# DecaYale/SYN3R

Measured on AMD Instinct MI355X. Metric: llff_3view_train_loop_iters_per_sec, higher is better.
Workload: dtype f32 raster / f16 UNet (f32 accumulate); 1 GPU; LLFF fern-like 3-view block: 50 raster fwd+bwd iters (l1 loss) (200000 Gaussians, 1920x1080, SH3) + 1 SVD (step,pass): CFG UNet fwd [2,14,8,72,128] f16 + fused Euler step; frames=14, parallelism=scene-parallel x1

## Files before the change

### syn3r_amd/csrc/raster_bin.hip

```cpp
#include "common.h"
#include "raster_common.h"

using namespace syn3r;

namespace syn3r {

size_t binning_bytes(long long P) {
    size_t n = (size_t)(P > 0 ? P : 1);
    return 2 * align256(n * 8) + 2 * align256(n * 4) + sort_scratch_bytes(n) + 256;
}

BinningState carve_binning(void* buf, long long P) {
    size_t n = (size_t)(P > 0 ? P : 1);
    char* p = (char*)buf;
    BinningState b;
    b.keys_a = (unsigned long long*)p; p += align256(n * 8);
    b.keys_b = (unsigned long long*)p; p += align256(n * 8);
    b.vals_a = (unsigned*)p; p += align256(n * 4);
    b.vals_b = (unsigned*)p; p += align256(n * 4);
    b.sort_scratch = p;
    return b;
}

}

namespace {

__global__ void __launch_bounds__(256) k_dup_tiles(int N, const unsigned* __restrict__ order,
                                                   const float* __restrict__ means2D, const int* __restrict__ radii,
                                                   const unsigned* __restrict__ offsets, int gx, int gy,
                                                   unsigned* __restrict__ keys, unsigned* __restrict__ vals,
                                                   unsigned cap, unsigned* __restrict__ header,
                                                   uint2* __restrict__ ranges, int tiles) {
    const int i = blockIdx.x * 256 + threadIdx.x;
    for (int t = i; t < tiles; t += gridDim.x * 256) ranges[t] = make_uint2(0u, 0u);
    const int lane = threadIdx.x & 63;
    const bool valid = i < N;
    unsigned id = valid ? order[i] : 0u;
    int r = valid ? radii[id] : 0;
    int x0 = 0, y0 = 0, x1 = 0, y1 = 0;
    if (r > 0) tile_rect(means2D[2 * (size_t)id], means2D[2 * (size_t)id + 1], r, gx, gy, x0, y0, x1, y1);
    const int w = x1 - x0;
    const unsigned cnt = (unsigned)(w * (y1 - y0));
    const unsigned incl = wave_scan_incl(cnt);
    const unsigned local = incl - cnt;
    const unsigned total = __shfl(incl, 63, 64);
    const int first = blockIdx.x * 256 + (threadIdx.x & ~63);
    const unsigned base = first < N ? offsets[first] : 0u;
    const float inv_w = w > 0 ? 1.0f / (float)w : 0.0f;
    for (unsigned t = 0; t < total; t += 64) {
        const unsigned p = t + lane;
        int j = 0;
#pragma unroll
        for (int step = 32; step > 0; step >>= 1) {
            unsigned lc = __shfl(local, j + step, 64);
            if (lc <= p) j += step;
        }
        const unsigned k = p - __shfl(local, j, 64);
        const int xj = __shfl(x0, j, 64), yj = __shfl(y0, j, 64), wj = __shfl(w, j, 64);
        const float iwj = __shfl(inv_w, j, 64);
        const unsigned idj = __shfl(id, j, 64);
        if (p < total) {
            const int ty = (int)(((float)k + 0.5f) * iwj);
            int tyc = ty;
            if ((unsigned)(tyc * wj) > k) --tyc;
            else if ((unsigned)((tyc + 1) * wj) <= k) ++tyc;
            const int tx = (int)k - tyc * wj;
            const unsigned o = base + p;
            if (o < cap) {
                keys[o] = (unsigned)((yj + tyc) * gx + xj + tx);
                vals[o] = idj;
            } else {
                header[1] = 1u;
// ... 491 lines not shown
```

### syn3r_amd/csrc/raster_bwd.hip

```cpp
#include "common.h"
#include "raster_common.h"

using namespace syn3r;

namespace {

constexpr int kGradSlots = 16;
enum { G_R = 0, G_G, G_B, G_DEPTH, G_MX, G_MY, G_CXX, G_CXY, G_CYY, G_OP, G_USED = 10 };

template <int NV>
__device__ __forceinline__ float reduce_lanes(float (&v)[10]) {
    static_assert(NV == 9 || NV == 10, "value 9 is the only optional one");
    float a[5];
#pragma unroll
    for (int k = 0; k < NV - 5; ++k) {
        auto r = __builtin_amdgcn_permlane32_swap(__float_as_int(v[k]), __float_as_int(v[k + 5]), false, false);
        a[k] = __int_as_float(r[0]) + __int_as_float(r[1]);
    }
    if (NV == 9) a[4] = v[4];
    float b[3];
#pragma unroll
    for (int k = 0; k < 2; ++k) {
        auto r = __builtin_amdgcn_permlane16_swap(__float_as_int(a[k]), __float_as_int(a[k + 3]), false, false);
        b[k] = __int_as_float(r[0]) + __int_as_float(r[1]);
    }
    b[2] = a[2];
    asm("s_nop 1\n\t"
        "v_add_f32_dpp %0, %0, %0 row_ror:8 row_mask:0xf bank_mask:0x3\n\t"
        "v_add_f32_dpp %0, %1, %1 row_ror:8 row_mask:0xf bank_mask:0xc\n\t"
        "v_add_f32_dpp %2, %2, %2 row_ror:8 row_mask:0xf bank_mask:0xf\n\t"
        "s_nop 0\n\t"
        "v_add_f32_dpp %0, %0, %0 row_ror:4 row_mask:0xf bank_mask:0xa\n\t"
        "v_add_f32_dpp %0, %2, %2 row_ror:4 row_mask:0xf bank_mask:0x5\n\t"
        "s_nop 1\n\t"
        "v_add_f32_dpp %0, %0, %0 row_ror:2 row_mask:0xf bank_mask:0xf\n\t"
        "s_nop 1\n\t"
        "v_add_f32_dpp %0, %0, %0 row_ror:1 row_mask:0xf bank_mask:0xf"
        : "+v"(b[0]), "+v"(b[1]), "+v"(b[2]));
    return b[0];
}
template <int NV>
__device__ __forceinline__ int reduce_value(int lane) {
    const int c = lane & 15, q = lane >> 4;
    if (c == 7) return ((5 * q + 1) >> 1);
    if (c == 15) return (NV == 9 && q == 3) ? 4 : ((5 * q + 1) >> 1) + 1;
    if (c == 3) return q < 2 ? 2 : 7;
    return -1;
}

constexpr int kBwdThreads = kBlendThreads;
#ifdef SYN3R_RASTER_STATS
__device__ unsigned long long g_bwd_stats[4];
#endif

template <bool HAS_DEPTH_GRAD>
__global__ void __launch_bounds__(kBwdThreads) k_render_bwd(
    int H, int W, int gx, int gy, const uint2* __restrict__ ranges, const unsigned* __restrict__ point_list,
    const Splat* __restrict__ splats, float bg0, float bg1, float bg2, const unsigned* __restrict__ n_contrib,
    const float* __restrict__ final_T, const float* __restrict__ dL_dcolor, const float* __restrict__ dL_ddepth,
    const float* __restrict__ dL_dalpha_out, float* __restrict__ grad_rec, const unsigned* __restrict__ tile_order) {
    __shared__ float4 sm[kBwdThreads * 3];
    __shared__ unsigned sid[kBwdThreads];
    __shared__ float sacc[kBwdThreads * kGradSlots];
    const unsigned tile = tile_order ? tile_order[blockIdx.x] : xcd_remap(blockIdx.x, (unsigned)(gx * gy));
    const int wq = threadIdx.x >> 6, lane = threadIdx.x & 63;
    const BlendFrame f = blend_frame(tile, wq, lane, H, W, gx);
    const bool in0 = f.in0, in1 = f.in1;
    const uint2 range = ranges[tile];
    const size_t hw = (size_t)H * W, pix0 = (size_t)f.py0 * W + f.px, pix1 = (size_t)f.py1 * W + f.px;

    const f2 T_final = (f2){in0 ? final_T[pix0] : 0.0f, in1 ? final_T[pix1] : 0.0f};
    f2 T = T_final;
    const int lc0 = in0 ? (int)n_contrib[pix0] : 0, lc1 = in1 ? (int)n_contrib[pix1] : 0;
    __shared__ int s_live;
    int wave_live;
    if (threadIdx.x == 0) s_live = 0;
    __syncthreads();
    {
        int mc = max(lc0, lc1);
#pragma unroll
        for (int o = 32; o > 0; o >>= 1) mc = max(mc, __shfl_xor(mc, o, 64));
        if (lane == 0) atomicMax(&s_live, mc);
        wave_live = mc;
    }
    __syncthreads();
    const int total = min(s_live, (int)(range.y - range.x));
    const int rounds = (total + kBwdThreads - 1) / kBwdThreads;
    const BlendHalf hf = blend_half(tile, wq, gx);
    f2 gr = splat2(0.f), gg = splat2(0.f), gb = splat2(0.f), gD = splat2(0.f), gA = splat2(0.f);
    if (in0) {
        gr.x = dL_dcolor[pix0]; gg.x = dL_dcolor[hw + pix0]; gb.x = dL_dcolor[2 * hw + pix0];
        if constexpr (HAS_DEPTH_GRAD) gD.x = dL_ddepth[pix0];
        gA.x = dL_dalpha_out ? dL_dalpha_out[pix0] : 0.0f;
    }
    if (in1) {
        gr.y = dL_dcolor[pix1]; gg.y = dL_dcolor[hw + pix1]; gb.y = dL_dcolor[2 * hw + pix1];
        if constexpr (HAS_DEPTH_GRAD) gD.y = dL_ddepth[pix1];
        gA.y = dL_dalpha_out ? dL_dalpha_out[pix1] : 0.0f;
    }
    const f2 tail = T_final * (gA - (bg0 * gr + bg1 * gg + bg2 * gb));
    f2 R = tail;

    constexpr int NV = HAS_DEPTH_GRAD ? 10 : 9;
    const int rval = reduce_value<NV>(lane);
    int rslot = -1;
    {
        const int order[10] = {G_R, G_G, G_B, G_MX, G_MY, G_CXX, G_CXY, G_CYY, G_OP, G_DEPTH};
#pragma unroll
        for (int k = 0; k < 10; ++k) rslot = rval == k ? order[k] : rslot;
    }
    int todo = total;
    float4 n0, n1, n2;
    unsigned ngid = 0;
    bool have = false;
    auto fetch = [&](int rd) {
        const int progress = rd * kBwdThreads + threadIdx.x;
        have = progress < total;
        if (have) {
            ngid = point_list[range.x + total - 1 - progress];
            const float4* src = (const float4*)(splats + ngid);
            n0 = src[0]; n1 = src[1]; n2 = src[2];
        }
    };
    fetch(0);
    for (int rd = 0; rd < rounds; ++rd, todo -= kBwdThreads) {
        __syncthreads();
        if (have) {
            stage_splat(sm, threadIdx.x, n0, n1, n2);
            sid[threadIdx.x] = ngid;
        }
        fetch(rd + 1);
#pragma unroll
        for (int k = 0; k < kGradSlots / 4; ++k)
            ((float4*)sacc)[threadIdx.x * (kGradSlots / 4) + k] = make_float4(0.f, 0.f, 0.f, 0.f);
        __syncthreads();
        const int cnt = min(kBwdThreads, todo);
        for (int c0 = 0; c0 < cnt; c0 += 64) {
          bool hit = false;
          if (c0 + lane < cnt) {
              const float4 ta = sm[(c0 + lane) * 3], tb = sm[(c0 + lane) * 3 + 1];
              hit = splat_reaches_rect(ta.x, ta.y, ta.z, ta.w, tb.x, tb.y, hf.sx0, hf.sx1, hf.sy0, hf.sy1) &&
                    (total - 1 - (rd * kBwdThreads + c0 + lane)) < wave_live;
          }
          unsigned long long vm = __ballot(hit);
          RASTER_STAT(g_bwd_stats, 0, min(64, cnt - c0));
          RASTER_STAT(g_bwd_stats, 1, __popcll(vm));
          while (vm) {
            const int j = c0 + (int)__builtin_ctzll(vm);
            vm &= vm - 1;
            const int contributor = total - 1 - (rd * kBwdThreads + j);
            const float4 a = sm[j * 3], b = sm[j * 3 + 1], c = sm[j * 3 + 2];
            const BlendEval e = blend_eval(a, b, f);
            const float dx = e.dx;
            const f2 dy = e.dy, power = e.power, araw = b.y * e.G;
            f2 G = e.G;
            const bool act0 = (contributor < lc0) && (power.x <= 0.0f) && (fminf(kAlphaMax, araw.x) >= kAlphaMin);
            const bool act1 = (contributor < lc1) && (power.y <= 0.0f) && (fminf(kAlphaMax, araw.y) >= kAlphaMin);
            if (__ballot(act0 || act1) == 0ull) continue;
            RASTER_STAT(g_bwd_stats, 2, 1); RASTER_STAT(g_bwd_stats, 3, __popcll(__ballot(act0)) + __popcll(__ballot(act1)));
            const f2 a_eff = (f2){act0 ? fminf(kAlphaMax, araw.x) : 0.0f, act1 ? fminf(kAlphaMax, araw.y) : 0.0f};
            G = (f2){act0 ? G.x : 0.0f, act1 ? G.y : 0.0f};
            const f2 one_m = 1.0f - a_eff;
            const f2 inv1ma = (f2){__builtin_amdgcn_rcpf(one_m.x), __builtin_amdgcn_rcpf(one_m.y)};
            T = T * inv1ma;
            const f2 wgt = a_eff * T;
            f2 d = b.z * gr;
            d = b.w * gg + d;
            d = c.x * gb + d;
            if constexpr (HAS_DEPTH_GRAD) d = c.y * gD + d;
            const f2 dL_da = T * d + inv1ma * R;
            R = R - wgt * d;
            const f2 h = G * dL_da;
            const f2 hy = h * dy, hyy = hy * dy;
            const f2 wr = wgt * gr, wg = wgt * gg, wb = wgt * gb;
            const float Sh = h.x + h.y, Sy = hy.x + hy.y, Sx = Sh * dx;
            float v[10];
            v[0] = wr.x + wr.y; v[1] = wg.x + wg.y; v[2] = wb.x + wb.y;
            v[3] = Sx;
            v[4] = Sy;
            v[5] = Sx * dx;
            v[6] = Sy * dx;
            v[7] = hyy.x + hyy.y;
            v[8] = Sh;
            v[9] = 0.0f;
            if constexpr (HAS_DEPTH_GRAD) { const f2 wd = wgt * gD; v[9] = wd.x + wd.y; }
            const float s = reduce_lanes<NV>(v);
            if (rslot >= 0) atomicAdd(&sacc[j * kGradSlots + rslot], s);
          }
        }
        __syncthreads();
        {
            const int slot = threadIdx.x & 15;
            for (int q = threadIdx.x >> 4; q < cnt; q += kBwdThreads / 16) {
                float val = sacc[q * kGradSlots + slot];
                if (slot < G_USED && val != 0.0f) unsafeAtomicAdd(grad_rec + (size_t)sid[q] * kGradSlots + slot, val);
            }
        }
    }
}

struct F3 { float x, y, z; };
__device__ __forceinline__ F3 f3(float x, float y, float z) { return {x, y, z}; }
__device__ __forceinline__ F3 operator*(float s, F3 a) { return {s * a.x, s * a.y, s * a.z}; }
// ... 224 lines not shown
        for (int k = 0; k < 12; ++k) {
            const int e = (threadIdx.x + 256 * k) * 4, row = e / 48, col = e - row * 48;
            if (row < rows) {
                const float* d = &shl[row * kShLd + col];
                *(float4*)(dL_dshs + blk0 + e) = make_float4(d[0], d[1], d[2], d[3]);
            }
        }
    }
}

}

extern "C" size_t syn3r_raster_backward_workspace_bytes(int N) {
    return N > 0 ? align256((size_t)N * kGradSlots * sizeof(float)) : 0;
}

static int raster_backward(int raw, int N, int sh_degree, int sh_coeffs, long long P, const float* means3D,
                                     const float* scales, const float* rotations, const float* opacities,
                                     const float* shs, const float* confidence, float scale_modifier,
                                     const float* viewmatrix, const float* projmatrix, const float* campos,
                                     float tanfovx, float tanfovy, int H, int W, const float* bg, const int* radii,
                                     void* geom, size_t geom_bytes_, const unsigned* point_list, void* image,
                                     size_t image_bytes_, const float* dL_dcolor, const float* dL_ddepth,
                                     const float* dL_dalpha, float* dL_dmeans3D, float* dL_dscales,
                                     float* dL_drotations, float* dL_dopacities, float* dL_dshs, float* dL_dmeans2D,
                                     float* dL_dconfidence, void* workspace, size_t workspace_bytes, void* stream_) {
    SYN3R_REQUIRE(N > 0 && H > 0 && W > 0 && P >= 0, "raster_backward: bad sizes N=%d H=%d W=%d P=%lld", N, H, W, P);
    SYN3R_REQUIRE(sh_degree >= 0 && sh_degree <= 3 && sh_coeffs >= (sh_degree + 1) * (sh_degree + 1),
                  "raster_backward: bad SH configuration");
    SYN3R_REQUIRE(means3D && scales && rotations && opacities && shs && viewmatrix && projmatrix && campos && bg && radii,
                  "raster_backward: null input");
    SYN3R_REQUIRE(dL_dcolor && dL_dmeans3D && dL_dscales && dL_drotations && dL_dopacities && dL_dshs && dL_dmeans2D,
                  "raster_backward: null gradient buffer");
    SYN3R_REQUIRE(P == 0 || point_list, "raster_backward: point list required");
    size_t need = syn3r_raster_backward_workspace_bytes(N);
    if (!geom || geom_bytes_ < geom_bytes(N) || !image || image_bytes_ < image_bytes(H, W) || !workspace ||
        workspace_bytes < need) {
        set_error("raster_backward: state/workspace buffer too small");
        return SYN3R_E_WORKSPACE;
    }
    hipStream_t stream = (hipStream_t)stream_;
    GeomState g = carve_geom(geom, N);
    ImageState im = carve_image(image, H, W);
    Camera cam;
    raster_fill_camera(cam, viewmatrix, projmatrix, campos, tanfovx, tanfovy, H, W);
    float* grad_rec = (float*)workspace;
    int rc = check_hip(hipMemsetAsync(grad_rec, 0, need, stream), "memset grads");
    if (rc) return rc;
    const unsigned tiles = (unsigned)(cam.grid_x * cam.grid_y);
    const unsigned* tile_order = raster_tiles_ordered(N, cam.grid_x, cam.grid_y) ? im.tile_order : nullptr;
    if (P > 0 && dL_ddepth)
        SYN3R_LAUNCH_NAMED("k_render_bwd", k_render_bwd<true>, dim3(tiles), dim3(kBwdThreads), 0, stream, H, W, cam.grid_x, cam.grid_y, im.ranges,
                           point_list, g.splats, bg[0], bg[1], bg[2], im.n_contrib, im.final_T, dL_dcolor, dL_ddepth,
                           dL_dalpha, grad_rec, tile_order);
    else if (P > 0)
        SYN3R_LAUNCH_NAMED("k_render_bwd", k_render_bwd<false>, dim3(tiles), dim3(kBwdThreads), 0, stream, H, W, cam.grid_x, cam.grid_y, im.ranges,
                           point_list, g.splats, bg[0], bg[1], bg[2], im.n_contrib, im.final_T, dL_dcolor, dL_ddepth,
                           dL_dalpha, grad_rec, tile_order);
    const bool staged = sh_coeffs == 16 && ((((uintptr_t)shs) | ((uintptr_t)dL_dshs)) & 15) == 0;
    if (staged)
        SYN3R_LAUNCH(k_preprocess_bwd<true>, dim3(ceil_div(N, 256)), dim3(256), 0, stream, N, sh_degree, sh_coeffs, means3D,
                       scales, rotations, opacities, shs, confidence, scale_modifier, cam, radii, g, grad_rec,
                       dL_dmeans3D, dL_dscales, dL_drotations, dL_dopacities, dL_dshs, dL_dmeans2D, dL_dconfidence, raw);
    else
        SYN3R_LAUNCH(k_preprocess_bwd<false>, dim3(ceil_div(N, 256)), dim3(256), 0, stream, N, sh_degree, sh_coeffs, means3D,
                       scales, rotations, opacities, shs, confidence, scale_modifier, cam, radii, g, grad_rec,
                       dL_dmeans3D, dL_dscales, dL_drotations, dL_dopacities, dL_dshs, dL_dmeans2D, dL_dconfidence, raw);
    SYN3R_LAUNCH_CHECK("raster_backward launch");
    return SYN3R_OK;
}

extern "C" int syn3r_raster_backward(int N, int sh_degree, int sh_coeffs, long long P, const float* means3D,
                                     const float* scales, const float* rotations, const float* opacities,
                                     const float* shs, const float* confidence, float scale_modifier,
                                     const float* viewmatrix, const float* projmatrix, const float* campos,
                                     float tanfovx, float tanfovy, int H, int W, const float* bg, const int* radii,
                                     void* geom, size_t geom_bytes_, const unsigned* point_list, void* image,
                                     size_t image_bytes_, const float* dL_dcolor, const float* dL_ddepth,
                                     const float* dL_dalpha, float* dL_dmeans3D, float* dL_dscales,
                                     float* dL_drotations, float* dL_dopacities, float* dL_dshs, float* dL_dmeans2D,
                                     float* dL_dconfidence, void* workspace, size_t workspace_bytes, void* stream_) {
    return raster_backward(0, N, sh_degree, sh_coeffs, P, means3D, scales, rotations, opacities, shs, confidence, scale_modifier,
                           viewmatrix, projmatrix, campos, tanfovx, tanfovy, H, W, bg, radii, geom, geom_bytes_, point_list, image,
                           image_bytes_, dL_dcolor, dL_ddepth, dL_dalpha, dL_dmeans3D, dL_dscales, dL_drotations, dL_dopacities,
                           dL_dshs, dL_dmeans2D, dL_dconfidence, workspace, workspace_bytes, stream_);
}

extern "C" int syn3r_raster_backward_raw(int N, int sh_degree, int sh_coeffs, long long P, const float* means3D,
                                         const float* log_scales, const float* raw_rotations, const float* opacity_logits,
                                         const float* shs, const float* confidence, float scale_modifier,
                                         const float* viewmatrix, const float* projmatrix, const float* campos,
                                         float tanfovx, float tanfovy, int H, int W, const float* bg, const int* radii,
                                         void* geom, size_t geom_bytes_, const unsigned* point_list, void* image,
                                         size_t image_bytes_, const float* dL_dcolor, const float* dL_ddepth,
                                         const float* dL_dalpha, float* dL_dmeans3D, float* dL_dlog_scales,
                                         float* dL_draw_rotations, float* dL_dopacity_logits, float* dL_dshs, float* dL_dmeans2D,
                                         float* dL_dconfidence, void* workspace, size_t workspace_bytes, void* stream_) {
    return raster_backward(1, N, sh_degree, sh_coeffs, P, means3D, log_scales, raw_rotations, opacity_logits, shs, confidence,
                           scale_modifier, viewmatrix, projmatrix, campos, tanfovx, tanfovy, H, W, bg, radii, geom, geom_bytes_,
                           point_list, image, image_bytes_, dL_dcolor, dL_ddepth, dL_dalpha, dL_dmeans3D, dL_dlog_scales,
                           dL_draw_rotations, dL_dopacity_logits, dL_dshs, dL_dmeans2D, dL_dconfidence, workspace, workspace_bytes,
                           stream_);
}

#ifdef SYN3R_RASTER_STATS
extern "C" __attribute__((visibility("default"))) int syn3r_debug_bwd_stats(unsigned long long* out4, int reset) {
    int rc = (int)hipMemcpyFromSymbol(out4, HIP_SYMBOL(g_bwd_stats), sizeof(unsigned long long) * 4);
    if (reset) { unsigned long long z[4] = {0, 0, 0, 0}; rc |= (int)hipMemcpyToSymbol(HIP_SYMBOL(g_bwd_stats), z, sizeof(z)); }
    return rc;
}
#endif
// ... 1 lines not shown
```

### syn3r_amd/csrc/raster_common.h

```cpp
#pragma once
#include <hip/hip_runtime.h>
#include <stdint.h>
#include <stddef.h>

namespace syn3r {

constexpr int kTileX = 16;
constexpr int kTileY = 16;
constexpr int kTilePix = kTileX * kTileY;
constexpr float kNearClip = 0.2f;
constexpr float kFovGuard = 1.3f;
constexpr float kLowPass = 0.3f;
constexpr float kAlphaMin = 1.0f / 255.0f;
constexpr float kAlphaMax = 0.99f;
constexpr float kTransmittanceMin = 1e-4f;
constexpr float kLog2e = 1.4426950408889634f;

struct alignas(16) Splat {
    float x, y;
    float cxx, cxy, cyy;
    float opacity;
    float r, g, b;
    float depth;
    float pad0, pad1;
};
static_assert(sizeof(Splat) == 48, "Splat must be 48 bytes");

struct GeomState {
    unsigned* header;
    float* depths;
    float* means2D;
    float* cov3D;
    float* conic_opacity;
    float* rgb;
    unsigned* clamped;
    unsigned* tiles_touched;
    unsigned* point_offsets;
    Splat* splats;
    unsigned* dkeys_a;
    unsigned* dkeys_b;
    unsigned* order_a;
    unsigned* order_b;
    unsigned* order;
    void* sort_scratch;
    void* scan_scratch;
};

#ifndef SYN3R_BIN_COUNTERS
#define SYN3R_BIN_COUNTERS 65536
#endif
constexpr size_t kBinCounters = SYN3R_BIN_COUNTERS;
constexpr size_t kMaxSuperSlots = 4096;
struct ImageState {
    uint2* ranges;
    unsigned* n_contrib;
    float* final_T;
    unsigned* tile_counts;
    unsigned* bin_counters;
    unsigned* tile_order;
};

struct BinningState {
    unsigned long long* keys_a;
    unsigned long long* keys_b;
    unsigned* vals_a;
    unsigned* vals_b;
    void* sort_scratch;
};

inline size_t align256(size_t x) { return (x + 255) & ~(size_t)255; }

size_t scan_scratch_bytes(size_t n);
size_t sort_scratch_bytes(size_t n);
int exclusive_scan_u32(const unsigned* in, unsigned* out, size_t n, unsigned* total_out, void* scratch,
                       hipStream_t stream, const unsigned* perm = nullptr);
int argsort_depth_u32(unsigned* keys_a, unsigned* vals_a, unsigned* keys_b, unsigned* vals_b, size_t n, void* scratch,
                      hipStream_t stream, int* result_in_b);
int sort_pairs_by_tile_u32(unsigned* keys_a, unsigned* vals_a, unsigned* keys_b, unsigned* vals_b, size_t n, int nbits,
                           void* scratch, hipStream_t stream, int* result_in_b, const unsigned* n_dev);
int radix_sort_pairs(unsigned long long* keys_a, unsigned* vals_a, unsigned long long* keys_b, unsigned* vals_b,
                     size_t n, int nbits, void* scratch, hipStream_t stream, int* result_in_b,
                     const unsigned* n_dev = nullptr);

struct Camera {
    float view[16];
    float proj[16];
    float campos[3];
    float tanfovx, tanfovy, focal_x, focal_y;
    int H, W, grid_x, grid_y;
};

size_t geom_bytes(int N);
bool raster_tiles_ordered(int N, int gx, int gy);
size_t image_bytes(int H, int W);
size_t binning_bytes(long long P);
GeomState carve_geom(void* buf, int N);
void raster_fill_camera(Camera& cam, const float* view, const float* proj, const float* campos, float tanfovx, float tanfovy, int H, int W);
ImageState carve_image(void* buf, int H, int W);
BinningState carve_binning(void* buf, long long P);

int raster_bin_prepare(const GeomState& g, int N, int gx, int gy, bool want_count, hipStream_t stream);
int raster_bin_lists(const GeomState& g, const ImageState& im, const BinningState& bn, const int* radii, int N, int gx, int gy,
                     long long P, hipStream_t stream, unsigned** point_list, const unsigned** tile_order);

#ifdef __HIPCC__
__device__ __forceinline__ bool splat_reaches_rect(float mx, float my, float A, float B, float C, float op, float x0,
                                                   float x1, float y0, float y1) {
    if (!(A > 0.0f && C > 0.0f)) return true;
    const float thr = 2.0f * __logf(255.0f * op);
    const float dx0 = x0 - mx, dx1 = x1 - mx, dy0 = y0 - my, dy1 = y1 - my;
    const bool inx = dx0 <= 0.0f && dx1 >= 0.0f, iny = dy0 <= 0.0f && dy1 >= 0.0f;
    float qmin = 0.0f;
    if (!(inx && iny)) {
        qmin = 3.0e38f;
        if (!inx) {
            const float dx = dx0 > 0.0f ? dx0 : dx1;
            const float dy = fminf(fmaxf(-B * dx / C, dy0), dy1);
            qmin = A * dx * dx + 2.0f * B * dx * dy + C * dy * dy;
        }
        if (!iny) {
            const float dy = dy0 > 0.0f ? dy0 : dy1;
// ... 97 lines not shown
```

### syn3r_amd/csrc/raster_fwd.hip

```cpp
#include "common.h"
#include "raster_common.h"

using namespace syn3r;

namespace syn3r {

size_t geom_bytes(int N) {
    size_t n = (size_t)N;
    size_t b = 256;
    b += align256(n * 4);
    b += align256(n * 8);
    b += align256(n * 24);
    b += align256(n * 16);
    b += align256(n * 12);
    b += align256(n * 4);
    b += align256(n * 4);
    b += align256(n * 4);
    b += align256(n * sizeof(Splat));
    b += 4 * align256(n * 4);
    b += align256(sort_scratch_bytes(n));
    b += scan_scratch_bytes(n);
    return b;
}

GeomState carve_geom(void* buf, int N) {
    size_t n = (size_t)N;
    char* p = (char*)buf;
    GeomState g;
    g.header = (unsigned*)p; p += 256;
    g.depths = (float*)p; p += align256(n * 4);
    g.means2D = (float*)p; p += align256(n * 8);
    g.cov3D = (float*)p; p += align256(n * 24);
    g.conic_opacity = (float*)p; p += align256(n * 16);
    g.rgb = (float*)p; p += align256(n * 12);
    g.clamped = (unsigned*)p; p += align256(n * 4);
    g.tiles_touched = (unsigned*)p; p += align256(n * 4);
    g.point_offsets = (unsigned*)p; p += align256(n * 4);
    g.splats = (Splat*)p; p += align256(n * sizeof(Splat));
    g.dkeys_a = (unsigned*)p; p += align256(n * 4);
    g.dkeys_b = (unsigned*)p; p += align256(n * 4);
    g.order_a = (unsigned*)p; p += align256(n * 4);
    g.order_b = (unsigned*)p; p += align256(n * 4);
    g.order = g.order_a;
    g.sort_scratch = p; p += align256(sort_scratch_bytes(n));
    g.scan_scratch = p;
    return g;
}

size_t image_bytes(int H, int W) {
    size_t tiles = (size_t)((W + kTileX - 1) / kTileX) * ((H + kTileY - 1) / kTileY);
    size_t px = (size_t)H * W;
    return align256(tiles * 8) + align256(px * 4) + align256(px * 4) + align256(tiles * 16) + align256((kBinCounters + kMaxSuperSlots) * 4) + align256(tiles * 4);
}

ImageState carve_image(void* buf, int H, int W) {
    size_t tiles = (size_t)((W + kTileX - 1) / kTileX) * ((H + kTileY - 1) / kTileY);
    size_t px = (size_t)H * W;
    char* p = (char*)buf;
    ImageState s;
    s.ranges = (uint2*)p; p += align256(tiles * 8);
    s.n_contrib = (unsigned*)p; p += align256(px * 4);
    s.final_T = (float*)p; p += align256(px * 4);
    s.tile_counts = (unsigned*)p; p += align256(tiles * 16);
    s.bin_counters = (unsigned*)p; p += align256((kBinCounters + kMaxSuperSlots) * 4);
    s.tile_order = (unsigned*)p;
    return s;
}


}

namespace {

__device__ __forceinline__ float3 xf43(const float* m, float3 p) {
    return make_float3(m[0] * p.x + m[4] * p.y + m[8] * p.z + m[12], m[1] * p.x + m[5] * p.y + m[9] * p.z + m[13],
                       m[2] * p.x + m[6] * p.y + m[10] * p.z + m[14]);
}
__device__ __forceinline__ float4 xf44(const float* m, float3 p) {
    return make_float4(m[0] * p.x + m[4] * p.y + m[8] * p.z + m[12], m[1] * p.x + m[5] * p.y + m[9] * p.z + m[13],
                       m[2] * p.x + m[6] * p.y + m[10] * p.z + m[14], m[3] * p.x + m[7] * p.y + m[11] * p.z + m[15]);
}

__device__ __forceinline__ float ndc2pix(float v, int S) { return ((v + 1.0f) * (float)S - 1.0f) * 0.5f; }

__device__ float3 sh_to_rgb(int D, int M, float3 pos, const float* campos, const float* __restrict__ sh,
                            unsigned& clamped) {
    float3 dir = make_float3(pos.x - campos[0], pos.y - campos[1], pos.z - campos[2]);
    float inv = 1.0f / sqrtf(dir.x * dir.x + dir.y * dir.y + dir.z * dir.z);
    dir.x *= inv; dir.y *= inv; dir.z *= inv;
    auto c = [&](int k) { return make_float3(sh[3 * k], sh[3 * k + 1], sh[3 * k + 2]); };
    auto mad = [](float3& a, float s, float3 b) { a.x += s * b.x; a.y += s * b.y; a.z += s * b.z; };
    float3 res = make_float3(0, 0, 0);
    mad(res, SH_C0, c(0));
    if (D > 0) {
        float x = dir.x, y = dir.y, z = dir.z;
        mad(res, -SH_C1 * y, c(1));
        mad(res, SH_C1 * z, c(2));
        mad(res, -SH_C1 * x, c(3));
        if (D > 1) {
            float xx = x * x, yy = y * y, zz = z * z, xy = x * y, yz = y * z, xz = x * z;
            mad(res, SH_C2[0] * xy, c(4));
            mad(res, SH_C2[1] * yz, c(5));
            mad(res, SH_C2[2] * (2.0f * zz - xx - yy), c(6));
            mad(res, SH_C2[3] * xz, c(7));
            mad(res, SH_C2[4] * (xx - yy), c(8));
            if (D > 2) {
                mad(res, SH_C3[0] * y * (3.0f * xx - yy), c(9));
                mad(res, SH_C3[1] * xy * z, c(10));
                mad(res, SH_C3[2] * y * (4.0f * zz - xx - yy), c(11));
                mad(res, SH_C3[3] * z * (2.0f * zz - 3.0f * xx - 3.0f * yy), c(12));
                mad(res, SH_C3[4] * x * (4.0f * zz - xx - yy), c(13));
                mad(res, SH_C3[5] * z * (xx - yy), c(14));
                mad(res, SH_C3[6] * x * (xx - 3.0f * yy), c(15));
            }
        }
    }
    res.x += 0.5f; res.y += 0.5f; res.z += 0.5f;
    clamped = (res.x < 0.0f ? 1u : 0u) | (res.y < 0.0f ? 2u : 0u) | (res.z < 0.0f ? 4u : 0u);
// ... 33 lines not shown
    float m20 = k.R20 * sx, m21 = k.R21 * sy, m22 = k.R22 * sz;
    float c0 = m00 * m00 + m01 * m01 + m02 * m02;
    float c1 = m00 * m10 + m01 * m11 + m02 * m12;
    float c2 = m00 * m20 + m01 * m21 + m02 * m22;
    float c3 = m10 * m10 + m11 * m11 + m12 * m12;
    float c4 = m10 * m20 + m11 * m21 + m12 * m22;
    float c5 = m20 * m20 + m21 * m21 + m22 * m22;
    float* cv = g.cov3D + 6 * (size_t)i;
    cv[0] = c0; cv[1] = c1; cv[2] = c2; cv[3] = c3; cv[4] = c4; cv[5] = c5;

    const EwaRows w = ewa_rows(cam, t.x, t.y, t.z);
    const float T00 = w.T00, T01 = w.T01, T02 = w.T02, T10 = w.T10, T11 = w.T11, T12 = w.T12;
    float a0 = c0 * T00 + c1 * T01 + c2 * T02, a1 = c1 * T00 + c3 * T01 + c4 * T02, a2 = c2 * T00 + c4 * T01 + c5 * T02;
    float b0 = c0 * T10 + c1 * T11 + c2 * T12, b1 = c1 * T10 + c3 * T11 + c4 * T12, b2 = c2 * T10 + c4 * T11 + c5 * T12;
    float cxx = T00 * a0 + T01 * a1 + T02 * a2 + kLowPass;
    float cxy = T00 * b0 + T01 * b1 + T02 * b2;
    float cyy = T10 * b0 + T11 * b1 + T12 * b2 + kLowPass;

    float det = cxx * cyy - cxy * cxy;
    if (det == 0.0f) return;
    float det_inv = 1.0f / det;
    float conx = cyy * det_inv, cony = -cxy * det_inv, conz = cxx * det_inv;
    float mid = 0.5f * (cxx + cyy);
    float sq = sqrtf(fmaxf(0.1f, mid * mid - det));
    float lambda1 = mid + sq, lambda2 = mid - sq;
    int radius = (int)ceilf(3.0f * sqrtf(fmaxf(lambda1, lambda2)));
    float px = ndc2pix(ndcx, cam.W), py = ndc2pix(ndcy, cam.H);
    int x0, y0, x1, y1;
    tile_rect(px, py, radius, cam.grid_x, cam.grid_y, x0, y0, x1, y1);
    int area = (x1 - x0) * (y1 - y0);
    if (area == 0) return;

    unsigned cl;
    float3 rgb = sh_to_rgb(D, M, p, cam.campos, shs + (size_t)i * M * 3, cl);
    float op = raw ? act_sigmoid(opacities[i]) : opacities[i];
    float cf = conf ? conf[i] : 1.0f;
    g.depths[i] = t.z;
    g.dkeys_a[i] = __float_as_uint(t.z);
    radii[i] = radius;
    g.means2D[2 * (size_t)i] = px;
    g.means2D[2 * (size_t)i + 1] = py;
    float* co = g.conic_opacity + 4 * (size_t)i;
    co[0] = conx; co[1] = cony; co[2] = conz; co[3] = op;
    g.rgb[3 * (size_t)i] = rgb.x; g.rgb[3 * (size_t)i + 1] = rgb.y; g.rgb[3 * (size_t)i + 2] = rgb.z;
    g.clamped[i] = cl;
    g.tiles_touched[i] = (unsigned)area;
    Splat s;
    s.x = px; s.y = py; s.cxx = conx; s.cxy = cony; s.cyy = conz; s.opacity = op * cf;
    s.r = rgb.x; s.g = rgb.y; s.b = rgb.z; s.depth = t.z; s.pad0 = 0.f; s.pad1 = 0.f;
    g.splats[i] = s;
}

constexpr int kFwdThreads = kBlendThreads;
#ifdef SYN3R_RASTER_STATS
__device__ unsigned long long g_fwd_stats[4];
#endif

__global__ void __launch_bounds__(kFwdThreads) k_render(int H, int W, int gx, int gy, const uint2* __restrict__ ranges,
                                                        const unsigned* __restrict__ point_list,
                                                        const Splat* __restrict__ splats, float bg0, float bg1,
                                                        float bg2, unsigned* __restrict__ n_contrib,
                                                        float* __restrict__ final_T, float* __restrict__ out_color,
                                                        float* __restrict__ out_depth, float* __restrict__ out_alpha,
                                                        const unsigned* __restrict__ tile_order) {
    __shared__ float4 sm[kFwdThreads * 3];
    const unsigned tile = tile_order ? tile_order[blockIdx.x] : xcd_remap(blockIdx.x, (unsigned)(gx * gy));
    const int wq = threadIdx.x >> 6, lane = threadIdx.x & 63;
    const BlendFrame f = blend_frame(tile, wq, lane, H, W, gx);
    const uint2 range = ranges[tile];
    const int total = (int)(range.y - range.x);
    const int rounds = (total + kFwdThreads - 1) / kFwdThreads;

    bool done0 = !f.in0, done1 = !f.in1;
    f2 T = (f2){1.0f, 1.0f}, Cr = (f2){0.f, 0.f}, Cg = Cr, Cb = Cr, Dp = Cr;
    unsigned last0 = 0, last1 = 0;
    int todo = total;
    const BlendHalf hf = blend_half(tile, wq, gx);
    float4 n0, n1, n2;
    bool have = false;
    auto fetch = [&](int rd) {
        const int idx = rd * kFwdThreads + threadIdx.x;
        have = idx < total;
        if (have) {
            const float4* src = (const float4*)(splats + point_list[range.x + idx]);
            n0 = src[0]; n1 = src[1]; n2 = src[2];
        }
    };
    fetch(0);
    for (int rd = 0; rd < rounds; ++rd, todo -= kFwdThreads) {
        if (__syncthreads_count(done0 && done1) == kFwdThreads) break;
        if (have) stage_splat(sm, threadIdx.x, n0, n1, n2);
        fetch(rd + 1);
        __syncthreads();
        const int cnt = min(kFwdThreads, todo);
        for (int c0 = 0; c0 < cnt; c0 += 64) {
            if (__ballot(!(done0 && done1)) == 0ull) break;
            bool hit = false;
            if (c0 + lane < cnt) {
                const float4 a = sm[(c0 + lane) * 3], b = sm[(c0 + lane) * 3 + 1];
                hit = splat_reaches_rect(a.x, a.y, a.z, a.w, b.x, b.y, hf.sx0, hf.sx1, hf.sy0, hf.sy1);
            }
            unsigned long long m = __ballot(hit);
            RASTER_STAT(g_fwd_stats, 0, min(64, cnt - c0));
            RASTER_STAT(g_fwd_stats, 1, __popcll(m));
            while (m) {
                const int j = c0 + (int)__builtin_ctzll(m);
                m &= m - 1;
                const float4 a = sm[j * 3], b = sm[j * 3 + 1], c = sm[j * 3 + 2];
                const BlendEval e = blend_eval(a, b, f);
                const f2 power = e.power, araw = b.y * e.G;
                const float al0 = fminf(kAlphaMax, araw.x), al1 = fminf(kAlphaMax, araw.y);
                const f2 w_raw = (f2){al0, al1} * T;
                const f2 test_T = T - w_raw;
                const bool c0_ = !done0 && power.x <= 0.0f && al0 >= kAlphaMin;
                const bool c1_ = !done1 && power.y <= 0.0f && al1 >= kAlphaMin;
                if (c0_ && test_T.x < kTransmittanceMin) done0 = true;
                if (c1_ && test_T.y < kTransmittanceMin) done1 = true;
                const bool t0 = c0_ && !done0, t1 = c1_ && !done1;
#ifdef SYN3R_RASTER_STATS
                { unsigned long long b0 = __ballot(t0), b1 = __ballot(t1); RASTER_STAT(g_fwd_stats, 2, (b0 | b1) != 0ull); RASTER_STAT(g_fwd_stats, 3, __popcll(b0) + __popcll(b1)); }
#endif
                const f2 w = (f2){t0 ? w_raw.x : 0.0f, t1 ? w_raw.y : 0.0f};
                Cr += b.z * w; Cg += b.w * w; Cb += c.x * w; Dp += c.y * w;
                T -= w;
                const unsigned here = (unsigned)(rd * kFwdThreads + j + 1);
                last0 = t0 ? here : last0;
                last1 = t1 ? here : last1;
            }
        }
    }
    const size_t hw = (size_t)H * W;
    if (f.in0) {
        const size_t pix = (size_t)f.py0 * W + f.px;
        final_T[pix] = T.x;
        n_contrib[pix] = last0;
        out_color[pix] = Cr.x + T.x * bg0;
        out_color[hw + pix] = Cg.x + T.x * bg1;
        out_color[2 * hw + pix] = Cb.x + T.x * bg2;
        out_depth[pix] = Dp.x;
        out_alpha[pix] = 1.0f - T.x;
    }
    if (f.in1) {
        const size_t pix = (size_t)f.py1 * W + f.px;
        final_T[pix] = T.y;
        n_contrib[pix] = last1;
        out_color[pix] = Cr.y + T.y * bg0;
        out_color[hw + pix] = Cg.y + T.y * bg1;
        out_color[2 * hw + pix] = Cb.y + T.y * bg2;
        out_depth[pix] = Dp.y;
        out_alpha[pix] = 1.0f - T.y;
    }
}

}

namespace syn3r {
void raster_fill_camera(Camera& cam, const float* view, const float* proj, const float* campos, float tanfovx,
                        float tanfovy, int H, int W) {
    for (int i = 0; i < 16; ++i) { cam.view[i] = view[i]; cam.proj[i] = proj[i]; }
    for (int i = 0; i < 3; ++i) cam.campos[i] = campos[i];
    cam.tanfovx = tanfovx; cam.tanfovy = tanfovy;
    cam.focal_x = W / (2.0f * tanfovx);
    cam.focal_y = H / (2.0f * tanfovy);
    cam.H = H; cam.W = W;
    cam.grid_x = (W + kTileX - 1) / kTileX;
    cam.grid_y = (H + kTileY - 1) / kTileY;
}
}

extern "C" size_t syn3r_raster_geom_bytes(int N) { return SYN3R_DIM_OK(N) ? geom_bytes(N) : 0; }
extern "C" size_t syn3r_raster_image_bytes(int H, int W) { return (SYN3R_SIDE_OK(H) && SYN3R_SIDE_OK(W)) ? image_bytes(H, W) : 0; }
extern "C" size_t syn3r_raster_binning_bytes(long long P) { return P >= 0 ? binning_bytes(P) : 0; }

static int raster_preprocess(int raw, int N, int sh_degree, int sh_coeffs, const float* means3D,
                             const float* scales, const float* rotations, const float* opacities,
                             const float* shs, const float* confidence, float scale_modifier,
                             const float* viewmatrix, const float* projmatrix, const float* campos,
                             float tanfovx, float tanfovy, int H, int W, int* radii, void* geom,
                             size_t geom_bytes_, long long* num_rendered_host, void* stream_) {
    SYN3R_REQUIRE(SYN3R_DIM_OK(N) && SYN3R_SIDE_OK(H) && SYN3R_SIDE_OK(W), "raster_preprocess: bad sizes N=%d H=%d W=%d", N, H, W);
// ... 23 lines not shown
        if (rc) return rc;
        rc = check_hip(hipStreamSynchronize(stream), "num_rendered sync");
        if (rc) return rc;
        *num_rendered_host = (long long)total;
    }
    return SYN3R_OK;
}

extern "C" int syn3r_raster_preprocess(int N, int sh_degree, int sh_coeffs, const float* means3D,
                                       const float* scales, const float* rotations, const float* opacities,
                                       const float* shs, const float* confidence, float scale_modifier,
                                       const float* viewmatrix, const float* projmatrix, const float* campos,
                                       float tanfovx, float tanfovy, int H, int W, int* radii, void* geom,
                                       size_t geom_bytes_, long long* num_rendered_host, void* stream_) {
    return raster_preprocess(0, N, sh_degree, sh_coeffs, means3D, scales, rotations, opacities, shs, confidence, scale_modifier,
                             viewmatrix, projmatrix, campos, tanfovx, tanfovy, H, W, radii, geom, geom_bytes_, num_rendered_host,
                             stream_);
}

extern "C" int syn3r_raster_preprocess_raw(int N, int sh_degree, int sh_coeffs, const float* means3D,
                                           const float* log_scales, const float* raw_rotations, const float* opacity_logits,
                                           const float* shs, const float* confidence, float scale_modifier,
                                           const float* viewmatrix, const float* projmatrix, const float* campos,
                                           float tanfovx, float tanfovy, int H, int W, int* radii, void* geom,
                                           size_t geom_bytes_, long long* num_rendered_host, void* stream_) {
    return raster_preprocess(1, N, sh_degree, sh_coeffs, means3D, log_scales, raw_rotations, opacity_logits, shs, confidence,
                             scale_modifier, viewmatrix, projmatrix, campos, tanfovx, tanfovy, H, W, radii, geom, geom_bytes_,
                             num_rendered_host, stream_);
}

extern "C" int syn3r_raster_render(int N, int H, int W, const float* bg, const int* radii, void* geom,
                                   size_t geom_bytes_, void* binning, size_t binning_bytes_, void* image,
                                   size_t image_bytes_, long long P, float* out_color, float* out_depth,
                                   float* out_alpha, unsigned** point_list_out, void* stream_) {
    SYN3R_REQUIRE(N > 0 && H > 0 && W > 0 && P >= 0 && P < (1ll << 31), "raster_render: bad sizes N=%d H=%d W=%d P=%lld",
                  N, H, W, P);
    SYN3R_REQUIRE(bg && radii && out_color && out_depth && out_alpha, "raster_render: null argument");
    if (!geom || geom_bytes_ < geom_bytes(N) || !image || image_bytes_ < image_bytes(H, W) || !binning ||
        binning_bytes_ < binning_bytes(P)) {
        set_error("raster_render: state buffer too small (geom %zu/%zu image %zu/%zu binning %zu/%zu)", geom_bytes_,
                  geom_bytes(N), image_bytes_, image_bytes(H, W), binning_bytes_, binning_bytes(P));
        return SYN3R_E_WORKSPACE;
    }
    hipStream_t stream = (hipStream_t)stream_;
    GeomState g = carve_geom(geom, N);
    ImageState im = carve_image(image, H, W);
    BinningState bn = carve_binning(binning, P);
    const int gx = (W + kTileX - 1) / kTileX, gy = (H + kTileY - 1) / kTileY;
    const size_t tiles = (size_t)gx * gy;
    unsigned* point_list = nullptr;
    const unsigned* tile_order = nullptr;
    if (int rc = raster_bin_lists(g, im, bn, radii, N, gx, gy, P, stream, &point_list, &tile_order)) return rc;
    SYN3R_LAUNCH(k_render, dim3((unsigned)tiles), dim3(kFwdThreads), 0, stream, H, W, gx, gy, im.ranges, point_list,
                       g.splats, bg[0], bg[1], bg[2], im.n_contrib, im.final_T, out_color, out_depth, out_alpha, tile_order);
    SYN3R_LAUNCH_CHECK("raster_render launch");
    if (point_list_out) *point_list_out = point_list;
    return SYN3R_OK;
}

#ifdef SYN3R_RASTER_STATS
extern "C" __attribute__((visibility("default"))) int syn3r_debug_fwd_stats(unsigned long long* out4, int reset) {
    int rc = (int)hipMemcpyFromSymbol(out4, HIP_SYMBOL(g_fwd_stats), sizeof(unsigned long long) * 4);
    if (reset) { unsigned long long z[4] = {0, 0, 0, 0}; rc |= (int)hipMemcpyToSymbol(HIP_SYMBOL(g_fwd_stats), z, sizeof(z)); }
    return rc;
}
#endif
```

Before: 411.7 iters/s.

## Record per-wave contributor bitmasks in forward and replay them in backward raster

The forward blend kernel now writes, for each wave and each 64-splat chunk, a bitmask of the splats that actually contributed to any pixel. These masks go to new per-tile and per-binning buffers. The backward kernel reads those masks instead of re-running the rect-overlap test and live-count check, so it skips splats that never contributed. The forward also keeps its done/take predicates as SGPR lane masks with inline cndmask asm. This adds global writes, extra workspace and a hidden pointer handoff through visit_link, and backward now depends on forward state from the same iteration.

```diff
diff --git a/syn3r_amd/csrc/raster_bin.hip b/syn3r_amd/csrc/raster_bin.hip
--- a/syn3r_amd/csrc/raster_bin.hip
+++ b/syn3r_amd/csrc/raster_bin.hip
@@ -7,7 +7,7 @@
 
 size_t binning_bytes(long long P) {
     size_t n = (size_t)(P > 0 ? P : 1);
-    return 2 * align256(n * 8) + 2 * align256(n * 4) + sort_scratch_bytes(n) + 256;
+    return 2 * align256(n * 8) + 2 * align256(n * 4) + align256(sort_scratch_bytes(n)) + 256 + align256(2 * visit_rest_words(P) * 8);
 }
 
 BinningState carve_binning(void* buf, long long P) {
@@ -18,7 +18,8 @@
     b.keys_b = (unsigned long long*)p; p += align256(n * 8);
     b.vals_a = (unsigned*)p; p += align256(n * 4);
     b.vals_b = (unsigned*)p; p += align256(n * 4);
-    b.sort_scratch = p;
+    b.sort_scratch = p; p += align256(sort_scratch_bytes(n)) + 256;
+    b.visit_rest = (unsigned long long*)p;
     return b;
 }
 
diff --git a/syn3r_amd/csrc/raster_bwd.hip b/syn3r_amd/csrc/raster_bwd.hip
--- a/syn3r_amd/csrc/raster_bwd.hip
+++ b/syn3r_amd/csrc/raster_bwd.hip
@@ -58,7 +58,8 @@
     int H, int W, int gx, int gy, const uint2* __restrict__ ranges, const unsigned* __restrict__ point_list,
     const Splat* __restrict__ splats, float bg0, float bg1, float bg2, const unsigned* __restrict__ n_contrib,
     const float* __restrict__ final_T, const float* __restrict__ dL_dcolor, const float* __restrict__ dL_ddepth,
-    const float* __restrict__ dL_dalpha_out, float* __restrict__ grad_rec, const unsigned* __restrict__ tile_order) {
+    const float* __restrict__ dL_dalpha_out, float* __restrict__ grad_rec, const unsigned* __restrict__ tile_order,
+    const unsigned long long* __restrict__ visit_first, const unsigned long long* __restrict__ visit_link) {
     __shared__ float4 sm[kBwdThreads * 3];
     __shared__ unsigned sid[kBwdThreads];
     __shared__ float sacc[kBwdThreads * kGradSlots];
@@ -81,12 +82,15 @@
 #pragma unroll
         for (int o = 32; o > 0; o >>= 1) mc = max(mc, __shfl_xor(mc, o, 64));
         if (lane == 0) atomicMax(&s_live, mc);
-        wave_live = mc;
+        wave_live = __builtin_amdgcn_readfirstlane(mc);
     }
     __syncthreads();
     const int total = min(s_live, (int)(range.y - range.x));
-    const int rounds = (total + kBwdThreads - 1) / kBwdThreads;
-    const BlendHalf hf = blend_half(tile, wq, gx);
+    const int top = (total + 63) & ~63;
+    const int rounds = (top + kBwdThreads - 1) / kBwdThreads;
+    const int wave_chunks = (min(wave_live, total) + 63) >> 6;
+    const unsigned long long* const vw_first = visit_first + (size_t)wq * (gx * gy) + tile;
+    const unsigned long long* const vw_rest = (const unsigned long long*)(uintptr_t)visit_link[0] + (size_t)wq * visit_link[1] + (range.x >> 6);
     f2 gr = splat2(0.f), gg = splat2(0.f), gb = splat2(0.f), gD = splat2(0.f), gA = splat2(0.f);
     if (in0) {
         gr.x = dL_dcolor[pix0]; gg.x = dL_dcolor[hw + pix0]; gb.x = dL_dcolor[2 * hw + pix0];
@@ -109,18 +113,22 @@
 #pragma unroll
         for (int k = 0; k < 10; ++k) rslot = rval == k ? order[k] : rslot;
     }
-    int todo = total;
+    int todo = top;
     float4 n0, n1, n2;
     unsigned ngid = 0;
     bool have = false;
+    unsigned long long nword = 0ull;
     auto fetch = [&](int rd) {
-        const int progress = rd * kBwdThreads + threadIdx.x;
-        have = progress < total;
+        const int entry = top - 1 - (rd * kBwdThreads + (int)threadIdx.x);
+        have = entry >= 0 && entry < total;
         if (have) {
-            ngid = point_list[range.x + total - 1 - progress];
+            ngid = point_list[range.x + entry];
             const float4* src = (const float4*)(splats + ngid);
             n0 = src[0]; n1 = src[1]; n2 = src[2];
         }
+        const int k = (top >> 6) - 1 - (rd * (kBwdThreads / 64) + (lane & 1));
+        nword = 0ull;
+        if (k >= 0 && k < wave_chunks) nword = *(k ? vw_rest + k : vw_first);
     };
     fetch(0);
     for (int rd = 0; rd < rounds; ++rd, todo -= kBwdThreads) {
@@ -129,6 +137,7 @@
             stage_splat(sm, threadIdx.x, n0, n1, n2);
             sid[threadIdx.x] = ngid;
         }
+        const unsigned long long word = nword;
         fetch(rd + 1);
 #pragma unroll
         for (int k = 0; k < kGradSlots / 4; ++k)
@@ -136,19 +145,13 @@
         __syncthreads();
         const int cnt = min(kBwdThreads, todo);
         for (int c0 = 0; c0 < cnt; c0 += 64) {
-          bool hit = false;
-          if (c0 + lane < cnt) {
-              const float4 ta = sm[(c0 + lane) * 3], tb = sm[(c0 + lane) * 3 + 1];
-              hit = splat_reaches_rect(ta.x, ta.y, ta.z, ta.w, tb.x, tb.y, hf.sx0, hf.sx1, hf.sy0, hf.sy1) &&
-                    (total - 1 - (rd * kBwdThreads + c0 + lane)) < wave_live;
-          }
-          unsigned long long vm = __ballot(hit);
-          RASTER_STAT(g_bwd_stats, 0, min(64, cnt - c0));
+          const unsigned wlo = __builtin_amdgcn_readlane((unsigned)word, c0 >> 6), whi = __builtin_amdgcn_readlane((unsigned)(word >> 32), c0 >> 6);
+          unsigned long long vm = __builtin_bitreverse64(((unsigned long long)whi << 32) | wlo);
           RASTER_STAT(g_bwd_stats, 1, __popcll(vm));
           while (vm) {
             const int j = c0 + (int)__builtin_ctzll(vm);
             vm &= vm - 1;
-            const int contributor = total - 1 - (rd * kBwdThreads + j);
+            const int contributor = top - 1 - (rd * kBwdThreads + j);
             const float4 a = sm[j * 3], b = sm[j * 3 + 1], c = sm[j * 3 + 2];
             const BlendEval e = blend_eval(a, b, f);
             const float dx = e.dx;
@@ -479,11 +482,11 @@
     if (P > 0 && dL_ddepth)
         SYN3R_LAUNCH_NAMED("k_render_bwd", k_render_bwd<true>, dim3(tiles), dim3(kBwdThreads), 0, stream, H, W, cam.grid_x, cam.grid_y, im.ranges,
                            point_list, g.splats, bg[0], bg[1], bg[2], im.n_contrib, im.final_T, dL_dcolor, dL_ddepth,
-                           dL_dalpha, grad_rec, tile_order);
+                           dL_dalpha, grad_rec, tile_order, im.visit_first, im.visit_link);
     else if (P > 0)
         SYN3R_LAUNCH_NAMED("k_render_bwd", k_render_bwd<false>, dim3(tiles), dim3(kBwdThreads), 0, stream, H, W, cam.grid_x, cam.grid_y, im.ranges,
                            point_list, g.splats, bg[0], bg[1], bg[2], im.n_contrib, im.final_T, dL_dcolor, dL_ddepth,
-                           dL_dalpha, grad_rec, tile_order);
+                           dL_dalpha, grad_rec, tile_order, im.visit_first, im.visit_link);
     const bool staged = sh_coeffs == 16 && ((((uintptr_t)shs) | ((uintptr_t)dL_dshs)) & 15) == 0;
     if (staged)
         SYN3R_LAUNCH(k_preprocess_bwd<true>, dim3(ceil_div(N, 256)), dim3(256), 0, stream, N, sh_degree, sh_coeffs, means3D,
diff --git a/syn3r_amd/csrc/raster_common.h b/syn3r_amd/csrc/raster_common.h
--- a/syn3r_amd/csrc/raster_common.h
+++ b/syn3r_amd/csrc/raster_common.h
@@ -58,6 +58,8 @@
     unsigned* tile_counts;
     unsigned* bin_counters;
     unsigned* tile_order;
+    unsigned long long* visit_first;
+    unsigned long long* visit_link;
 };
 
 struct BinningState {
@@ -66,7 +68,9 @@
     unsigned* vals_a;
     unsigned* vals_b;
     void* sort_scratch;
-};
+    unsigned long long* visit_rest;
+};
+inline size_t visit_rest_words(long long P) { return (size_t)(P > 0 ? P : 1) / 64 + 2; }
 
 inline size_t align256(size_t x) { return (x + 255) & ~(size_t)255; }
 
diff --git a/syn3r_amd/csrc/raster_fwd.hip b/syn3r_amd/csrc/raster_fwd.hip
--- a/syn3r_amd/csrc/raster_fwd.hip
+++ b/syn3r_amd/csrc/raster_fwd.hip
@@ -50,7 +50,8 @@
 size_t image_bytes(int H, int W) {
     size_t tiles = (size_t)((W + kTileX - 1) / kTileX) * ((H + kTileY - 1) / kTileY);
     size_t px = (size_t)H * W;
-    return align256(tiles * 8) + align256(px * 4) + align256(px * 4) + align256(tiles * 16) + align256((kBinCounters + kMaxSuperSlots) * 4) + align256(tiles * 4);
+    return align256(tiles * 8) + align256(px * 4) + align256(px * 4) + align256(tiles * 16) + align256((kBinCounters + kMaxSuperSlots) * 4) + align256(tiles * 4) +
+           align256(2 * tiles * 8) + 256;
 }
 
 ImageState carve_image(void* buf, int H, int W) {
@@ -63,7 +64,9 @@
     s.final_T = (float*)p; p += align256(px * 4);
     s.tile_counts = (unsigned*)p; p += align256(tiles * 16);
     s.bin_counters = (unsigned*)p; p += align256((kBinCounters + kMaxSuperSlots) * 4);
-    s.tile_order = (unsigned*)p;
+    s.tile_order = (unsigned*)p; p += align256(tiles * 4);
+    s.visit_first = (unsigned long long*)p; p += align256(2 * tiles * 8);
+    s.visit_link = (unsigned long long*)p;
     return s;
 }
 
@@ -203,6 +206,18 @@
 }
 
 constexpr int kFwdThreads = kBlendThreads;
+typedef unsigned long long lanemask;
+enum { kCmpGE = 3, kCmpLT = 4, kCmpLE = 5 };
+__device__ __forceinline__ float take_or_zero(lanemask m, float a) {
+    float r;
+    asm("v_cndmask_b32_e64 %0, 0, %1, %2" : "=v"(r) : "v"(a), "s"(m));
+    return r;
+}
+__device__ __forceinline__ unsigned take_or_keep(lanemask m, unsigned a, unsigned b) {
+    unsigned r;
+    asm("v_cndmask_b32_e64 %0, %1, %2, %3" : "=v"(r) : "v"(b), "v"(a), "s"(m));
+    return r;
+}
 #ifdef SYN3R_RASTER_STATS
 __device__ unsigned long long g_fwd_stats[4];
 #endif
@@ -213,7 +228,10 @@
                                                         float bg2, unsigned* __restrict__ n_contrib,
                                                         float* __restrict__ final_T, float* __restrict__ out_color,
                                                         float* __restrict__ out_depth, float* __restrict__ out_alpha,
-                                                        const unsigned* __restrict__ tile_order) {
+                                                        const unsigned* __restrict__ tile_order,
+                                                        unsigned long long* __restrict__ visit_first,
+                                                        unsigned long long* __restrict__ visit_rest, unsigned visit_stride,
+                                                        unsigned long long* __restrict__ visit_link) {
     __shared__ float4 sm[kFwdThreads * 3];
     const unsigned tile = tile_order ? tile_order[blockIdx.x] : xcd_remap(blockIdx.x, (unsigned)(gx * gy));
     const int wq = threadIdx.x >> 6, lane = threadIdx.x & 63;
@@ -221,8 +239,12 @@
     const uint2 range = ranges[tile];
     const int total = (int)(range.y - range.x);
     const int rounds = (total + kFwdThreads - 1) / kFwdThreads;
-
-    bool done0 = !f.in0, done1 = !f.in1;
+    if (blockIdx.x == 0 && threadIdx.x == 0) { visit_link[0] = (unsigned long long)(uintptr_t)visit_rest; visit_link[1] = visit_stride; }
+    const unsigned wq_u = __builtin_amdgcn_readfirstlane(wq), tile_u = __builtin_amdgcn_readfirstlane(tile);
+    unsigned long long* const vw_first = visit_first + (wq_u * (unsigned)(gx * gy) + tile_u);
+    unsigned long long* const vw_rest = visit_rest + (wq_u * visit_stride + (__builtin_amdgcn_readfirstlane(range.x) >> 6));
+
+    lanemask done0 = __ballot(!f.in0), done1 = __ballot(!f.in1);
     f2 T = (f2){1.0f, 1.0f}, Cr = (f2){0.f, 0.f}, Cg = Cr, Cb = Cr, Dp = Cr;
     unsigned last0 = 0, last1 = 0;
     int todo = total;
@@ -239,23 +261,25 @@
     };
     fetch(0);
     for (int rd = 0; rd < rounds; ++rd, todo -= kFwdThreads) {
-        if (__syncthreads_count(done0 && done1) == kFwdThreads) break;
+        if (__syncthreads_count((done0 & done1) == ~0ull) == kFwdThreads) break;
         if (have) stage_splat(sm, threadIdx.x, n0, n1, n2);
         fetch(rd + 1);
         __syncthreads();
         const int cnt = min(kFwdThreads, todo);
         for (int c0 = 0; c0 < cnt; c0 += 64) {
-            if (__ballot(!(done0 && done1)) == 0ull) break;
+            if ((done0 & done1) == ~0ull) break;
             bool hit = false;
             if (c0 + lane < cnt) {
                 const float4 a = sm[(c0 + lane) * 3], b = sm[(c0 + lane) * 3 + 1];
                 hit = splat_reaches_rect(a.x, a.y, a.z, a.w, b.x, b.y, hf.sx0, hf.sx1, hf.sy0, hf.sy1);
             }
             unsigned long long m = __ballot(hit);
+            unsigned long long took = 0ull;
             RASTER_STAT(g_fwd_stats, 0, min(64, cnt - c0));
             RASTER_STAT(g_fwd_stats, 1, __popcll(m));
             while (m) {
                 const int j = c0 + (int)__builtin_ctzll(m);
+                const unsigned long long jbit = m & (0ull - m);
                 m &= m - 1;
                 const float4 a = sm[j * 3], b = sm[j * 3 + 1], c = sm[j * 3 + 2];
                 const BlendEval e = blend_eval(a, b, f);
@@ -263,20 +287,25 @@
                 const float al0 = fminf(kAlphaMax, araw.x), al1 = fminf(kAlphaMax, araw.y);
                 const f2 w_raw = (f2){al0, al1} * T;
                 const f2 test_T = T - w_raw;
-                const bool c0_ = !done0 && power.x <= 0.0f && al0 >= kAlphaMin;
-                const bool c1_ = !done1 && power.y <= 0.0f && al1 >= kAlphaMin;
-                if (c0_ && test_T.x < kTransmittanceMin) done0 = true;
-                if (c1_ && test_T.y < kTransmittanceMin) done1 = true;
-                const bool t0 = c0_ && !done0, t1 = c1_ && !done1;
+                const lanemask c0_ = ~done0 & __builtin_amdgcn_fcmpf(power.x, 0.0f, kCmpLE) & __builtin_amdgcn_fcmpf(al0, kAlphaMin, kCmpGE);
+                const lanemask c1_ = ~done1 & __builtin_amdgcn_fcmpf(power.y, 0.0f, kCmpLE) & __builtin_amdgcn_fcmpf(al1, kAlphaMin, kCmpGE);
+                done0 |= c0_ & __builtin_amdgcn_fcmpf(test_T.x, kTransmittanceMin, kCmpLT);
+                done1 |= c1_ & __builtin_amdgcn_fcmpf(test_T.y, kTransmittanceMin, kCmpLT);
+                const lanemask t0 = c0_ & ~done0, t1 = c1_ & ~done1;
+                if (t0 | t1) took |= jbit;
 #ifdef SYN3R_RASTER_STATS
-                { unsigned long long b0 = __ballot(t0), b1 = __ballot(t1); RASTER_STAT(g_fwd_stats, 2, (b0 | b1) != 0ull); RASTER_STAT(g_fwd_stats, 3, __popcll(b0) + __popcll(b1)); }
+                { unsigned long long b0 = t0, b1 = t1; RASTER_STAT(g_fwd_stats, 2, (b0 | b1) != 0ull); RASTER_STAT(g_fwd_stats, 3, __popcll(b0) + __popcll(b1)); }
 #endif
-                const f2 w = (f2){t0 ? w_raw.x : 0.0f, t1 ? w_raw.y : 0.0f};
+                const f2 w = (f2){take_or_zero(t0, w_raw.x), take_or_zero(t1, w_raw.y)};
                 Cr += b.z * w; Cg += b.w * w; Cb += c.x * w; Dp += c.y * w;
                 T -= w;
                 const unsigned here = (unsigned)(rd * kFwdThreads + j + 1);
-                last0 = t0 ? here : last0;
-                last1 = t1 ? here : last1;
+                last0 = take_or_keep(t0, here, last0);
+                last1 = take_or_keep(t1, here, last1);
+            }
+            if (lane == 0) {
+                const int k = rd * (kFwdThreads / 64) + (c0 >> 6);
+                if (k) vw_rest[k] = took; else *vw_first = took;
             }
         }
     }
@@ -406,7 +435,8 @@
     const unsigned* tile_order = nullptr;
     if (int rc = raster_bin_lists(g, im, bn, radii, N, gx, gy, P, stream, &point_list, &tile_order)) return rc;
     SYN3R_LAUNCH(k_render, dim3((unsigned)tiles), dim3(kFwdThreads), 0, stream, H, W, gx, gy, im.ranges, point_list,
-                       g.splats, bg[0], bg[1], bg[2], im.n_contrib, im.final_T, out_color, out_depth, out_alpha, tile_order);
+                       g.splats, bg[0], bg[1], bg[2], im.n_contrib, im.final_T, out_color, out_depth, out_alpha, tile_order,
+                       im.visit_first, bn.visit_rest, (unsigned)visit_rest_words(P), im.visit_link);
     SYN3R_LAUNCH_CHECK("raster_render launch");
     if (point_list_out) *point_list_out = point_list;
     return SYN3R_OK;
```

Result: no change. 413.1 iters/s, median of 6 (+0.4%).
